# KinWaiCheuk/ReconVAT

Hardware: AMD Instinct MI355X
Metric: training audio-sec/sec (node) (higher is better)
Workload: dtype f32; 1 GPU; ReconVAT UNet_Onset VAT=True reconstruction=True, per-GPU B_l=8 + B_ul=8 segments of 327680 samples (640 frames x 229 mel), Adam+StepLR, fp32; parallelism=dp1, hipgraph=True, two_stream_schedule=True, kernel_plan_table=644fe159bb9eb70e, kernel_plan_mode=table, vat_nan_flag=0

## Files before the change

reconvat_amd/csrc/bn.hip:

```cpp
#include "common.h"

#define BN_PIX_PER_THREAD 16

__device__ __forceinline__ float bn_momentum_update(float running, float batch, float momentum) {
    return __fmaf_rn(momentum, batch, __fmul_rn(1.f - momentum, running));
}

struct BnArgs {
    const float* z; int z_ld;
    const float* dy; int dy_ld;
    float* out; int out_ld;
    const float* res; int res_ld;
    const float* r1_x; int r1_x_ld; const float* r1_w; const float* r1_b; int sk_cin, sk_ks;
    long P; int C;
    double* sums;
    const float* coef;
    float slope;
    int frozen;
    float* dgamma; float* dbeta;
    int accumulate;
    int param_accumulate;
    const float* gamma; const float* beta;
    float* running_mean; float* running_var; long* nbt;
    float* coef_out;
    float momentum, eps;
    int training;
    int ppt;
};

template <bool BWD>
__global__ __launch_bounds__(256) void bn_reduce_k(BnArgs a) {
    __shared__ float sh[256 * 8];
    const int C = a.C, C4 = C >> 2, PL = 256 / C4;
    const int t = threadIdx.x;
    const int c = (t % C4) * 4, pl = t / C4;
    f32x4 s0 = (f32x4){0.f, 0.f, 0.f, 0.f}, s1 = (f32x4){0.f, 0.f, 0.f, 0.f};
    if (pl < PL) {
        const long p0 = (long)blockIdx.x * PL * a.ppt;
        f32x4 mean, invstd, scale, shift;
        if (BWD) {
            mean = *reinterpret_cast<const f32x4*>(a.coef + c);
            invstd = *reinterpret_cast<const f32x4*>(a.coef + C + c);
            scale = *reinterpret_cast<const f32x4*>(a.coef + 2 * C + c);
            shift = *reinterpret_cast<const f32x4*>(a.coef + 3 * C + c);
        }
        for (int k = 0; k < a.ppt; k += 4) {
            f32x4 zv[4], dv[4];
            bool ok[4];
#pragma unroll
            for (int u = 0; u < 4; ++u) {
                const long p = p0 + pl + (long)(k + u) * PL;
                ok[u] = p < a.P;
                const long pp = ok[u] ? p : 0;
                zv[u] = *reinterpret_cast<const f32x4*>(a.z + pp * a.z_ld + c);
                if (BWD) dv[u] = *reinterpret_cast<const f32x4*>(a.dy + pp * a.dy_ld + c);
            }
#pragma unroll
            for (int u = 0; u < 4; ++u) {
                if (!ok[u]) continue;
                const f32x4 z = zv[u];
                if (BWD) {
                    const f32x4 d = dv[u];
#pragma unroll
                    for (int q = 0; q < 4; ++q) {
                        float zh = fmaf(z[q], scale[q], shift[q]);
                        float dd = zh > 0.f ? d[q] : d[q] * a.slope;
                        s0[q] += dd;
                        s1[q] += dd * ((z[q] - mean[q]) * invstd[q]);
                    }
                } else {
                    s0 += z;
#pragma unroll
                    for (int q = 0; q < 4; ++q) s1[q] = fmaf(z[q], z[q], s1[q]);
                }
            }
        }
    }
    if (pl < PL) {
#pragma unroll
        for (int q = 0; q < 4; ++q) {
            sh[(pl * C + c + q) * 2] = s0[q];
            sh[(pl * C + c + q) * 2 + 1] = s1[q];
        }
    }
    __syncthreads();
    if (t < 2 * C) {
        const int ch = t >> 1, which = t & 1;
        double d = 0.0;
        for (int l = 0; l < PL; ++l) d += (double)sh[(l * C + ch) * 2 + which];
        atomicAdd(&a.sums[(blockIdx.x % RV_BN_NREP) * 2 * C + which * C + ch], d);
    }
}

__device__ __forceinline__ void bn_coef(const BnArgs& a, const double* fold, int c, float& mean, float& invstd) {
    if (a.training) {
        const double n = (double)a.P;
        const double m = fold[c] / n;
        double var = fold[a.C + c] / n - m * m;
        if (var < 0.0) var = 0.0;
        mean = (float)m;
        invstd = (float)(1.0 / sqrt(var + (double)a.eps));
    } else {
        mean = a.running_mean[c];
        invstd = 1.0f / sqrtf(a.running_var[c] + a.eps);
    }
}

template <bool BWD, int SKIP = 0>
__global__ __launch_bounds__(256) void bn_apply_k(BnArgs a) {
    static_assert(!BWD || SKIP == 0, "the fused skip conv exists in the forward kernel only");
    extern __shared__ __attribute__((aligned(16))) float skw[];
    const int C = a.C, C4 = C >> 2;
    const long total = a.P * C4;
    const long stride = (long)gridDim.x * blockDim.x;
    long idx = (long)blockIdx.x * blockDim.x + threadIdx.x;
    const bool fixed = (stride % C4) == 0;
    int c = (int)(idx % C4) * 4;
    __shared__ double fold[256];
    if (BWD ? !a.frozen || a.dgamma : a.training) {
        for (int i = threadIdx.x; i < 2 * C; i += blockDim.x) fold[i] = bn_sum_replicas(a.sums, C, i);
        __syncthreads();
    }
    f32x4 mean, invstd, scale, shift, k1, k2;
    auto fetch = [&](int cc) {
        if (BWD) {
            scale = *reinterpret_cast<const f32x4*>(a.coef + 2 * C + cc);
            shift = *reinterpret_cast<const f32x4*>(a.coef + 3 * C + cc);
            mean = *reinterpret_cast<const f32x4*>(a.coef + cc);
            invstd = *reinterpret_cast<const f32x4*>(a.coef + C + cc);
            const double invn = 1.0 / (double)a.P;
#pragma unroll
            for (int q = 0; q < 4; ++q) {
                k1[q] = a.frozen ? 0.f : (float)(fold[cc + q] * invn);
                k2[q] = a.frozen ? 0.f : (float)(fold[C + cc + q] * invn);
            }
        } else {
#pragma unroll
            for (int q = 0; q < 4; ++q) {
                float m_, is_;
                bn_coef(a, fold, cc + q, m_, is_);
                scale[q] = a.gamma[cc + q] * is_;
                shift[q] = a.beta[cc + q] - m_ * scale[q];
            }
        }
    };
    fetch(c);
    f32x4 r1w = (f32x4){0.f, 0.f, 0.f, 0.f}, r1b = (f32x4){0.f, 0.f, 0.f, 0.f};
    auto fetch_r1 = [&](int cc) {
        if (!BWD && a.r1_x) {
            if (SKIP == 0) r1w = *reinterpret_cast<const f32x4*>(a.r1_w + cc);
            if (a.r1_b) r1b = *reinterpret_cast<const f32x4*>(a.r1_b + cc);
        }
    };
    fetch_r1(c);
    if constexpr (SKIP > 0) {
        for (int i = threadIdx.x; i < SKIP * C; i += blockDim.x) {
            const int cc = i / SKIP, kk = i - cc * SKIP;
            skw[kk * C + cc] = a.r1_w[i];
        }
        __syncthreads();
    }
    auto skip_dense = [&](const long p, const int cc0) -> f32x4 {
        constexpr int NCH = SKIP > 0 ? SKIP / 16 : 1;
        const float* xp = a.r1_x + p * a.r1_x_ld;
        auto chunk = [&](f32x4& acc, const int ch) {
            f32x4 xg[4];
#pragma unroll
            for (int g = 0; g < 4; ++g) xg[g] = *reinterpret_cast<const f32x4*>(xp + 16 * ch + 4 * g);
#pragma unroll
            for (int r = 0; r < 4; ++r)
#pragma unroll
                for (int g = 0; g < 4; ++g) {
                    const f32x4 w4 = *reinterpret_cast<const f32x4*>(&skw[(16 * ch + 4 * g + r) * C + cc0]);
#pragma unroll
                    for (int q = 0; q < 4; ++q) acc[q] = fmaf(w4[q], xg[g][r], acc[q]);
                }
        };
        f32x4 tot = (f32x4){0.f, 0.f, 0.f, 0.f};
        if (!a.sk_ks) {
#pragma unroll
            for (int ch = 0; ch < NCH; ++ch) chunk(tot, ch);
        } else {
#pragma unroll
            for (int w = 0; w < 4; ++w) {
                f32x4 part = (f32x4){0.f, 0.f, 0.f, 0.f};
                for (int ch = (w * NCH) / 4; ch < ((w + 1) * NCH) / 4; ++ch) chunk(part, ch);
                if (w == 0) tot = part; else tot += part;
            }
        }
        return tot + r1b;
    };
    auto one = [&](const f32x4& z, const f32x4& d, const f32x4& r) -> f32x4 {
        f32x4 o;
        if (!BWD) {
#pragma unroll
            for (int q = 0; q < 4; ++q) {
                float zh = fmaf(z[q], scale[q], shift[q]);
                o[q] = (zh > 0.f ? zh : zh * a.slope) + r[q];
            }
        } else {
#pragma unroll
            for (int q = 0; q < 4; ++q) {
                float zh = fmaf(z[q], scale[q], shift[q]);
                float dz = zh > 0.f ? d[q] : d[q] * a.slope;
                float xh = (z[q] - mean[q]) * invstd[q];
                dz = dz - k1[q] - xh * k2[q];
                o[q] = dz * scale[q];
            }
        }
        return o;
    };
    if (fixed) {
        constexpr int UNR = BWD || SKIP > 0 ? 4 : 8;
        const long pstep = stride / C4;
        long p = idx / C4;
        for (; p < a.P; p += UNR * pstep) {
            f32x4 zv[UNR], dv[UNR], rv[UNR];
            bool ok[UNR];
#pragma unroll
            for (int u = 0; u < UNR; ++u) {
                const long pu = p + u * pstep;
                ok[u] = pu < a.P;
                const long pp = ok[u] ? pu : 0;
                zv[u] = *reinterpret_cast<const f32x4*>(a.z + pp * a.z_ld + c);
                if (BWD) dv[u] = *reinterpret_cast<const f32x4*>(a.dy + pp * a.dy_ld + c);
                else dv[u] = (f32x4){0.f, 0.f, 0.f, 0.f};
                rv[u] = (f32x4){0.f, 0.f, 0.f, 0.f};
                if (!BWD && a.res) rv[u] = *reinterpret_cast<const f32x4*>(a.res + pp * a.res_ld + c);
                if (!BWD && SKIP == 0 && a.r1_x) {
                    const float x1 = a.r1_x[pp * a.r1_x_ld];
#pragma unroll
                    for (int q = 0; q < 4; ++q) rv[u][q] = fmaf(x1, r1w[q], r1b[q]);
                }
            }
            if constexpr (SKIP > 0) {
#pragma unroll
                for (int u = 0; u < UNR; ++u) rv[u] = skip_dense(ok[u] ? p + u * pstep : 0, c);
            }
#pragma unroll
            for (int u = 0; u < UNR; ++u) {
                if (!ok[u]) continue;
                f32x4 o = one(zv[u], dv[u], rv[u]);
                float* dst = a.out + (p + u * pstep) * a.out_ld + c;
                if (a.accumulate) {
                    f32x4 old = *reinterpret_cast<f32x4*>(dst);
                    o += old;
                }
                *reinterpret_cast<f32x4*>(dst) = o;
            }
        }
        idx = total;
    }
    for (; idx < total; idx += stride) {
        const long p = idx / C4;
        if (!fixed) { c = (int)(idx - p * C4) * 4; fetch(c); fetch_r1(c); }
        const f32x4 z = *reinterpret_cast<const f32x4*>(a.z + p * a.z_ld + c);
        f32x4 o;
        if (!BWD) {
            f32x4 r = (f32x4){0.f, 0.f, 0.f, 0.f};
            if (a.res) r = *reinterpret_cast<const f32x4*>(a.res + p * a.res_ld + c);
            if (SKIP == 0 && a.r1_x) {
                const float x1 = a.r1_x[p * a.r1_x_ld];
#pragma unroll
                for (int q = 0; q < 4; ++q) r[q] = fmaf(x1, r1w[q], r1b[q]);
            }
            if constexpr (SKIP > 0) r = skip_dense(p, c);
#pragma unroll
            for (int q = 0; q < 4; ++q) {
                float zh = fmaf(z[q], scale[q], shift[q]);
                o[q] = (zh > 0.f ? zh : zh * a.slope) + r[q];
            }
        } else {
            const f32x4 d = *reinterpret_cast<const f32x4*>(a.dy + p * a.dy_ld + c);
#pragma unroll
            for (int q = 0; q < 4; ++q) {
                float zh = fmaf(z[q], scale[q], shift[q]);
                float dz = zh > 0.f ? d[q] : d[q] * a.slope;
                float xh = (z[q] - mean[q]) * invstd[q];
                dz = dz - k1[q] - xh * k2[q];
                o[q] = dz * scale[q];
            }
        }
        float* dst = a.out + p * a.out_ld + c;
        if (a.accumulate) {
            f32x4 old = *reinterpret_cast<f32x4*>(dst);
            o += old;
        }
        *reinterpret_cast<f32x4*>(dst) = o;
    }
    if (blockIdx.x == 0) {
        for (int cc = threadIdx.x; cc < a.C; cc += blockDim.x) {
            if (BWD) {
                if (a.dgamma) {
                    const float dg = (float)fold[a.C + cc], db = (float)fold[cc];
                    a.dgamma[cc] = a.param_accumulate ? a.dgamma[cc] + dg : dg;
                    a.dbeta[cc] = a.param_accumulate ? a.dbeta[cc] + db : db;
                }
            } else {
                float m_, is_;
                bn_coef(a, fold, cc, m_, is_);
                const float sc = a.gamma[cc] * is_;
                a.coef_out[cc] = m_;
                a.coef_out[a.C + cc] = is_;
                a.coef_out[2 * a.C + cc] = sc;
                a.coef_out[3 * a.C + cc] = a.beta[cc] - m_ * sc;
                if (a.training) {
                    const double n = (double)a.P;
                    const double mm = fold[cc] / n;
                    double var = fold[a.C + cc] / n - mm * mm;
                    if (var < 0.0) var = 0.0;
                    const float unb = (float)(n > 1.0 ? var * n / (n - 1.0) : var);
                    a.coef_out[4 * a.C + cc] = unb;
                    if (a.training == 1) {
                        a.running_mean[cc] = bn_momentum_update(a.running_mean[cc], m_, a.momentum);
                        a.running_var[cc] = bn_momentum_update(a.running_var[cc], unb, a.momentum);
                    }
                }
            }
        }
        if (!BWD && threadIdx.x == 0 && a.training == 1 && a.nbt) *a.nbt += 1;
    }
}

static int bn_apply_blocks(long total, bool bwd = false) {
    long b = (total + 255) / 256;
    static const long capf = getenv("RV_BN_MAXBLK") ? atol(getenv("RV_BN_MAXBLK")) : 768;
    static const long capb = getenv("RV_BN_MAXBLK_BWD") ? atol(getenv("RV_BN_MAXBLK_BWD")) : 768;
    const long cap = bwd ? capb : capf;
    if (b > cap) b = cap;
    b = ((b + 2) / 3) * 3;
    return (int)b;
}

static int bn_ppt(long P, int PL) {
    long ppt = P / ((long)PL * 512);
    ppt = (ppt + 3) & ~3L;
    if (ppt < BN_PIX_PER_THREAD) ppt = BN_PIX_PER_THREAD;
    if (ppt > 256) ppt = 256;
    return (int)ppt;
}

int rv_internal_bn_stats(const float* z, int z_ld, long P, int C, double* sums, hipStream_t st) {
    RV_CHECK_ARG(C % 4 == 0 && C <= 128 && (z_ld % 4) == 0, "bn statistics: C=%d must be a multiple of 4 and <= 128", C);
    BnArgs a = {};
    a.z = z; a.z_ld = z_ld; a.P = P; a.C = C; a.sums = sums;
    const int PL = 256 / (C / 4);
    a.ppt = bn_ppt(P, PL);
    hipLaunchKernelGGL(bn_reduce_k<false>, dim3(cdiv(P, (long)PL * a.ppt)), dim3(256), 0, st, a);
    RV_LAUNCH_CHECK("bn statistics");
    return RV_OK;
}

int rv_internal_bn_bwd_stats(const float* dy, int dy_ld, const float* z, int z_ld, long P, int C, const float* coef, float slope,
                             double* sums, hipStream_t st) {
    RV_CHECK_ARG(C % 4 == 0 && C <= 128 && (z_ld % 4) == 0 && (dy_ld % 4) == 0, "bn backward statistics: C=%d unsupported", C);
    BnArgs a = {};
    a.z = z; a.z_ld = z_ld; a.dy = dy; a.dy_ld = dy_ld; a.P = P; a.C = C; a.sums = sums; a.coef = coef; a.slope = slope;
    const int PL = 256 / (C / 4);
    a.ppt = bn_ppt(P, PL);
    hipLaunchKernelGGL(bn_reduce_k<true>, dim3(cdiv(P, (long)PL * a.ppt)), dim3(256), 0, st, a);
    RV_LAUNCH_CHECK("bn backward statistics");
    return RV_OK;
}

extern "C" {

long rv_bn_workspace_bytes(int C) { return (long)RV_BN_NREP * (2 * C) * 8; }

int rv_bn_lrelu_fwd(const float* z, int z_ld, long P, int C, const float* gamma, const float* beta, float* running_mean,
                    float* running_var, long* num_batches_tracked, float momentum, float eps, int training, float slope,
                    const float* res, int res_ld, float* y, int y_ld, float* coef, void* workspace, int sums_ready,
                    void* stream) {
    hipStream_t st = (hipStream_t)stream;
    RV_CHECK_ARG(C % 4 == 0 && C <= 128, "rv_bn_lrelu_fwd: C=%d must be a multiple of 4 and <= 128", C);
    RV_CHECK_ARG((z_ld % 4) == 0 && (y_ld % 4) == 0 && (!res || (res_ld % 4) == 0), "rv_bn_lrelu_fwd: strides must be multiples of 4");
    BnArgs a = {};
    a.z = z; a.z_ld = z_ld; a.P = P; a.C = C; a.sums = (double*)workspace; a.slope = slope;
    a.gamma = gamma; a.beta = beta; a.running_mean = running_mean; a.running_var = running_var; a.nbt = num_batches_tracked;
    a.coef_out = coef; a.momentum = momentum; a.eps = eps; a.training = training;
    if (training && !sums_ready) {
        const int rc = rv_internal_bn_stats(z, z_ld, P, C, a.sums, st);
        if (rc != RV_OK) return rc;
    }
    a.out = y; a.out_ld = y_ld; a.res = res; a.res_ld = res_ld;
    hipLaunchKernelGGL(bn_apply_k<false>, dim3(bn_apply_blocks(P * (C / 4))), dim3(256), 0, st, a);
    RV_LAUNCH_CHECK("rv_bn_lrelu_fwd(apply)");
    return RV_OK;
}

int rv_bn_lrelu_fwd_skip(const float* z, int z_ld, long P, int C, const float* gamma, const float* beta, float* running_mean,
                         float* running_var, long* num_batches_tracked, float momentum, float eps, int training, float slope,
                         const float* x, int x_ld, int cin, const float* w, const float* b, int ksplit, float* y, int y_ld, float* coef,
                         void* workspace, int sums_ready, void* stream) {
    hipStream_t st = (hipStream_t)stream;
    RV_CHECK_ARG(C % 4 == 0 && C <= 128, "rv_bn_lrelu_fwd_skip: C=%d must be a multiple of 4 and <= 128", C);
    RV_CHECK_ARG(cin == 1 || cin == 16 || cin == 32 || cin == 64, "rv_bn_lrelu_fwd_skip: cin=%d (1, 16, 32 or 64)", cin);
    RV_CHECK_ARG((z_ld % 4) == 0 && (y_ld % 4) == 0 && x && w && x_ld >= cin && (cin == 1 || ((x_ld % 4) == 0 && (((uintptr_t)x) & 15) == 0)),
                 "rv_bn_lrelu_fwd_skip: bad strides / alignment / null skip operands");
    BnArgs a = {};
    a.z = z; a.z_ld = z_ld; a.P = P; a.C = C; a.sums = (double*)workspace; a.slope = slope;
    a.gamma = gamma; a.beta = beta; a.running_mean = running_mean; a.running_var = running_var; a.nbt = num_batches_tracked;
    a.coef_out = coef; a.momentum = momentum; a.eps = eps; a.training = training;
    if (training && !sums_ready) {
        const int rc = rv_internal_bn_stats(z, z_ld, P, C, a.sums, st);
        if (rc != RV_OK) return rc;
    }
    a.out = y; a.out_ld = y_ld; a.r1_x = x; a.r1_x_ld = x_ld; a.r1_w = w; a.r1_b = b; a.sk_cin = cin; a.sk_ks = ksplit;
    const dim3 grid(bn_apply_blocks(P * (C / 4)));
    const size_t lds = (size_t)cin * C * sizeof(float);
    if (cin == 1) hipLaunchKernelGGL((bn_apply_k<false, 0>), grid, dim3(256), 0, st, a);
    else if (cin == 16) hipLaunchKernelGGL((bn_apply_k<false, 16>), grid, dim3(256), lds, st, a);
    else if (cin == 32) hipLaunchKernelGGL((bn_apply_k<false, 32>), grid, dim3(256), lds, st, a);
    else hipLaunchKernelGGL((bn_apply_k<false, 64>), grid, dim3(256), lds, st, a);
    RV_LAUNCH_CHECK("rv_bn_lrelu_fwd_skip(apply)");
    return RV_OK;
}

int rv_bn_lrelu_bwd(const float* dy, int dy_ld, const float* z, int z_ld, long P, int C, const float* coef, float slope,
                    int frozen, float* dz, int dz_ld, float* dgamma, float* dbeta, int param_accumulate, void* workspace,
                    int sums_ready, void* stream) {
    hipStream_t st = (hipStream_t)stream;
    RV_CHECK_ARG(C % 4 == 0 && C <= 128, "rv_bn_lrelu_bwd: C=%d must be a multiple of 4 and <= 128", C);
    BnArgs a = {};
    a.z = z; a.z_ld = z_ld; a.dy = dy; a.dy_ld = dy_ld; a.P = P; a.C = C; a.sums = (double*)workspace;
    a.coef = coef; a.slope = slope; a.frozen = frozen; a.out = dz; a.out_ld = dz_ld; a.dgamma = dgamma; a.dbeta = dbeta; a.param_accumulate = param_accumulate;
    if ((!frozen || dgamma) && !sums_ready) {
        const int rc = rv_internal_bn_bwd_stats(dy, dy_ld, z, z_ld, P, C, coef, slope, a.sums, st);
        if (rc != RV_OK) return rc;
    }
    hipLaunchKernelGGL(bn_apply_k<true>, dim3(bn_apply_blocks(P * (C / 4), true)), dim3(256), 0, st, a);
    RV_LAUNCH_CHECK("rv_bn_lrelu_bwd(apply)");
    return RV_OK;
}

__global__ void bn_running_update_k(float* rm, float* rv, long* nbt, const float* coef, int C, float momentum) {
    int c = blockIdx.x * blockDim.x + threadIdx.x;
    if (c == 0 && nbt) *nbt += 1;
    if (c >= C) return;
    rm[c] = bn_momentum_update(rm[c], coef[c], momentum);
    rv[c] = bn_momentum_update(rv[c], coef[4 * C + c], momentum);
}

__global__ __launch_bounds__(128) void bn_running_update_table_k(const long* table, int nlayers, float momentum) {
    const long* e = table + (long)blockIdx.x * 6;
    float* rm = (float*)e[0];
    float* rv = (float*)e[1];
    long* nbt = (long*)e[2];
    const int C = (int)e[3];
    const long first = e[4], count = e[5];
    const long* coefs = table + (long)nlayers * 6 + first;
    for (int c = threadIdx.x; c < C; c += blockDim.x) {
        float m = rm[c], v = rv[c];
        for (long k = 0; k < count; ++k) {
            const float* coef = (const float*)coefs[k];
            m = bn_momentum_update(m, coef[c], momentum);
            v = bn_momentum_update(v, coef[4 * C + c], momentum);
        }
        rm[c] = m; rv[c] = v;
    }
    if (threadIdx.x == 0 && nbt) *nbt += count;
}

int rv_bn_running_update_table(const long* table, int nlayers, float momentum, void* stream) {
    RV_CHECK_ARG(table && nlayers > 0, "rv_bn_running_update_table: empty table");
    hipLaunchKernelGGL(bn_running_update_table_k, dim3(nlayers), dim3(128), 0, (hipStream_t)stream, table, nlayers, momentum);
    RV_LAUNCH_CHECK("rv_bn_running_update_table");
    return RV_OK;
}

int rv_bn_running_update(float* running_mean, float* running_var, long* num_batches_tracked, const float* coef, int C,
                         float momentum, void* stream) {
    hipLaunchKernelGGL(bn_running_update_k, dim3(cdiv(C, 128)), dim3(128), 0, (hipStream_t)stream, running_mean, running_var,
                       num_batches_tracked, coef, C, momentum);
    RV_LAUNCH_CHECK("rv_bn_running_update");
    return RV_OK;
}

}
```

Measured before the change: 16560 audio-s/s.

## Overlap BN apply prologue with first tile loads via per-channel coefficient table

Restructures the BN apply kernel prologue. The first unrolled batch of activation loads is issued before the replica-sum reduction, and one thread per channel computes scale/shift (or k1/k2) once into an LDS table instead of every thread recomputing them per channel. Block 0 can also finalize coef_out and running stats early, and the residual and skip variants become template parameters to remove runtime branches. The cost is raw s_barrier inline asm and more register pressure from holding the loads live across the reduction.

```diff
diff --git a/reconvat_amd/csrc/bn.hip b/reconvat_amd/csrc/bn.hip
--- a/reconvat_amd/csrc/bn.hip
+++ b/reconvat_amd/csrc/bn.hip
@@ -92,65 +92,70 @@
     }
 }
 
-__device__ __forceinline__ void bn_coef(const BnArgs& a, const double* fold, int c, float& mean, float& invstd) {
+__device__ __forceinline__ void bn_coef(const BnArgs& a, double sum, double sumsq, float rmean, float rvar, float& mean, float& invstd) {
     if (a.training) {
         const double n = (double)a.P;
-        const double m = fold[c] / n;
-        double var = fold[a.C + c] / n - m * m;
+        const double m = sum / n;
+        double var = sumsq / n - m * m;
         if (var < 0.0) var = 0.0;
         mean = (float)m;
         invstd = (float)(1.0 / sqrt(var + (double)a.eps));
     } else {
-        mean = a.running_mean[c];
-        invstd = 1.0f / sqrtf(a.running_var[c] + a.eps);
-    }
-}
-
-template <bool BWD, int SKIP = 0>
+        mean = rmean;
+        invstd = 1.0f / sqrtf(rvar + a.eps);
+    }
+}
+
+#ifndef RV_BN_HEAD
+#define RV_BN_HEAD 3
+#endif
+
+template <bool BWD, int SKIP = 0, int RES = 0>
 __global__ __launch_bounds__(256) void bn_apply_k(BnArgs a) {
-    static_assert(!BWD || SKIP == 0, "the fused skip conv exists in the forward kernel only");
+    static_assert(!BWD || (SKIP == 0 && RES == 0), "residual and fused skip conv exist in the forward kernel only");
+    static_assert(SKIP == 0 || RES == 0, "the dense skip conv is the residual");
+    constexpr bool HOIST = (RV_BN_HEAD & 1) != 0, EARLY = (RV_BN_HEAD & 2) != 0;
     extern __shared__ __attribute__((aligned(16))) float skw[];
+    __shared__ double fold[256];
+    __shared__ __attribute__((aligned(16))) float ctab[256];
     const int C = a.C, C4 = C >> 2;
     const long total = a.P * C4;
     const long stride = (long)gridDim.x * blockDim.x;
     long idx = (long)blockIdx.x * blockDim.x + threadIdx.x;
     const bool fixed = (stride % C4) == 0;
     int c = (int)(idx % C4) * 4;
-    __shared__ double fold[256];
-    if (BWD ? !a.frozen || a.dgamma : a.training) {
-        for (int i = threadIdx.x; i < 2 * C; i += blockDim.x) fold[i] = bn_sum_replicas(a.sums, C, i);
-        __syncthreads();
+    const int tc = threadIdx.x;
+    const bool coef_thread = tc < C;
+    const bool sums = BWD ? !a.frozen || a.dgamma : a.training != 0;
+    double rep[RV_BN_NREP];
+    float gam = 0.f, bet = 0.f, rmean = 0.f, rvar = 0.f;
+    if (sums && tc < 2 * C) {
+#pragma unroll
+        for (int r = 0; r < RV_BN_NREP; ++r) rep[r] = a.sums[r * 2 * C + tc];
+    }
+    if (!BWD && coef_thread) {
+        gam = a.gamma[tc];
+        bet = a.beta[tc];
+        if (!a.training) { rmean = a.running_mean[tc]; rvar = a.running_var[tc]; }
     }
     f32x4 mean, invstd, scale, shift, k1, k2;
-    auto fetch = [&](int cc) {
+    auto fetch_saved = [&](int cc) {
         if (BWD) {
             scale = *reinterpret_cast<const f32x4*>(a.coef + 2 * C + cc);
             shift = *reinterpret_cast<const f32x4*>(a.coef + 3 * C + cc);
             mean = *reinterpret_cast<const f32x4*>(a.coef + cc);
             invstd = *reinterpret_cast<const f32x4*>(a.coef + C + cc);
-            const double invn = 1.0 / (double)a.P;
-#pragma unroll
-            for (int q = 0; q < 4; ++q) {
-                k1[q] = a.frozen ? 0.f : (float)(fold[cc + q] * invn);
-                k2[q] = a.frozen ? 0.f : (float)(fold[C + cc + q] * invn);
-            }
-        } else {
-#pragma unroll
-            for (int q = 0; q < 4; ++q) {
-                float m_, is_;
-                bn_coef(a, fold, cc + q, m_, is_);
-                scale[q] = a.gamma[cc + q] * is_;
-                shift[q] = a.beta[cc + q] - m_ * scale[q];
-            }
-        }
-    };
-    fetch(c);
+        }
+    };
+    auto fetch_table = [&](int cc) {
+        const f32x4 t0 = *reinterpret_cast<const f32x4*>(&ctab[cc]), t1 = *reinterpret_cast<const f32x4*>(&ctab[C + cc]);
+        if (BWD) { k1 = t0; k2 = t1; } else { scale = t0; shift = t1; }
+    };
+    fetch_saved(c);
     f32x4 r1w = (f32x4){0.f, 0.f, 0.f, 0.f}, r1b = (f32x4){0.f, 0.f, 0.f, 0.f};
     auto fetch_r1 = [&](int cc) {
-        if (!BWD && a.r1_x) {
-            if (SKIP == 0) r1w = *reinterpret_cast<const f32x4*>(a.r1_w + cc);
-            if (a.r1_b) r1b = *reinterpret_cast<const f32x4*>(a.r1_b + cc);
-        }
+        if (RES == 2) r1w = *reinterpret_cast<const f32x4*>(a.r1_w + cc);
+        if ((RES == 2 || SKIP > 0) && a.r1_b) r1b = *reinterpret_cast<const f32x4*>(a.r1_b + cc);
     };
     fetch_r1(c);
     if constexpr (SKIP > 0) {
@@ -158,8 +163,8 @@
             const int cc = i / SKIP, kk = i - cc * SKIP;
             skw[kk * C + cc] = a.r1_w[i];
         }
-        __syncthreads();
-    }
+    }
+    asm volatile("" ::: "memory");
     auto skip_dense = [&](const long p, const int cc0) -> f32x4 {
         constexpr int NCH = SKIP > 0 ? SKIP / 16 : 1;
         const float* xp = a.r1_x + p * a.r1_x_ld;
@@ -210,116 +215,149 @@
         }
         return o;
     };
-    if (fixed) {
-        constexpr int UNR = BWD || SKIP > 0 ? 4 : 8;
-        const long pstep = stride / C4;
-        long p = idx / C4;
-        for (; p < a.P; p += UNR * pstep) {
-            f32x4 zv[UNR], dv[UNR], rv[UNR];
-            bool ok[UNR];
+    constexpr int UNR = BWD || SKIP > 0 ? 4 : 8;
+    const long pstep = stride / C4;
+    long p = idx / C4;
+    f32x4 zv[UNR], dv[UNR], rv[UNR];
+    bool ok[UNR];
+    auto load_trip = [&]() __attribute__((always_inline)) {
+#pragma unroll
+        for (int u = 0; u < UNR; ++u) {
+            const long pu = p + u * pstep;
+            ok[u] = pu < a.P;
+            const long pp = ok[u] ? pu : 0;
+            zv[u] = *reinterpret_cast<const f32x4*>(a.z + pp * a.z_ld + c);
+            if (BWD) dv[u] = *reinterpret_cast<const f32x4*>(a.dy + pp * a.dy_ld + c);
+            else dv[u] = (f32x4){0.f, 0.f, 0.f, 0.f};
+            rv[u] = (f32x4){0.f, 0.f, 0.f, 0.f};
+            if (RES == 1) rv[u] = *reinterpret_cast<const f32x4*>(a.res + pp * a.res_ld + c);
+            if (RES == 2) rv[u][0] = a.r1_x[pp * a.r1_x_ld];
+        }
+    };
+    auto finish_trip = [&]() __attribute__((always_inline)) {
+        if (RES == 2) {
 #pragma unroll
             for (int u = 0; u < UNR; ++u) {
-                const long pu = p + u * pstep;
-                ok[u] = pu < a.P;
-                const long pp = ok[u] ? pu : 0;
-                zv[u] = *reinterpret_cast<const f32x4*>(a.z + pp * a.z_ld + c);
-                if (BWD) dv[u] = *reinterpret_cast<const f32x4*>(a.dy + pp * a.dy_ld + c);
-                else dv[u] = (f32x4){0.f, 0.f, 0.f, 0.f};
-                rv[u] = (f32x4){0.f, 0.f, 0.f, 0.f};
-                if (!BWD && a.res) rv[u] = *reinterpret_cast<const f32x4*>(a.res + pp * a.res_ld + c);
-                if (!BWD && SKIP == 0 && a.r1_x) {
-                    const float x1 = a.r1_x[pp * a.r1_x_ld];
-#pragma unroll
-                    for (int q = 0; q < 4; ++q) rv[u][q] = fmaf(x1, r1w[q], r1b[q]);
+                const float x1 = rv[u][0];
+#pragma unroll
+                for (int q = 0; q < 4; ++q) rv[u][q] = fmaf(x1, r1w[q], r1b[q]);
+            }
+        }
+        if constexpr (SKIP > 0) {
+#pragma unroll
+            for (int u = 0; u < UNR; ++u) rv[u] = skip_dense(ok[u] ? p + u * pstep : 0, c);
+        }
+#pragma unroll
+        for (int u = 0; u < UNR; ++u) {
+            if (!ok[u]) continue;
+            f32x4 o = one(zv[u], dv[u], rv[u]);
+            float* dst = a.out + (p + u * pstep) * a.out_ld + c;
+            if (a.accumulate) {
+                f32x4 old = *reinterpret_cast<f32x4*>(dst);
+                o += old;
+            }
+            *reinterpret_cast<f32x4*>(dst) = o;
+        }
+    };
+    double s0 = 0.0, s1 = 0.0;
+    auto finalize = [&]() {
+        if (BWD) {
+            if (a.dgamma) {
+                const float dg = (float)s1, db = (float)s0;
+                a.dgamma[tc] = a.param_accumulate ? a.dgamma[tc] + dg : dg;
+                a.dbeta[tc] = a.param_accumulate ? a.dbeta[tc] + db : db;
+            }
+        } else {
+            float m_, is_;
+            bn_coef(a, s0, s1, rmean, rvar, m_, is_);
+            const float sc = gam * is_;
+            a.coef_out[tc] = m_;
+            a.coef_out[C + tc] = is_;
+            a.coef_out[2 * C + tc] = sc;
+            a.coef_out[3 * C + tc] = bet - m_ * sc;
+            if (a.training) {
+                const double n = (double)a.P;
+                const double mm = s0 / n;
+                double var = s1 / n - mm * mm;
+                if (var < 0.0) var = 0.0;
+                const float unb = (float)(n > 1.0 ? var * n / (n - 1.0) : var);
+                a.coef_out[4 * C + tc] = unb;
+                if (a.training == 1) {
+                    a.running_mean[tc] = bn_momentum_update(a.running_mean[tc], m_, a.momentum);
+                    a.running_var[tc] = bn_momentum_update(a.running_var[tc], unb, a.momentum);
                 }
             }
-            if constexpr (SKIP > 0) {
-#pragma unroll
-                for (int u = 0; u < UNR; ++u) rv[u] = skip_dense(ok[u] ? p + u * pstep : 0, c);
-            }
-#pragma unroll
-            for (int u = 0; u < UNR; ++u) {
-                if (!ok[u]) continue;
-                f32x4 o = one(zv[u], dv[u], rv[u]);
-                float* dst = a.out + (p + u * pstep) * a.out_ld + c;
-                if (a.accumulate) {
-                    f32x4 old = *reinterpret_cast<f32x4*>(dst);
-                    o += old;
+            if (tc == 0 && a.training == 1 && a.nbt) *a.nbt += 1;
+        }
+    };
+    auto head = [&]() __attribute__((always_inline)) {
+        if (sums) {
+            if (tc < 2 * C) {
+                double s = 0.0;
+#pragma unroll
+                for (int r = 0; r < RV_BN_NREP; ++r) {
+                    asm volatile("" : "+v"(rep[r]));
+                    s += rep[r];
                 }
-                *reinterpret_cast<f32x4*>(dst) = o;
-            }
-        }
-        idx = total;
-    }
-    for (; idx < total; idx += stride) {
-        const long p = idx / C4;
-        if (!fixed) { c = (int)(idx - p * C4) * 4; fetch(c); fetch_r1(c); }
-        const f32x4 z = *reinterpret_cast<const f32x4*>(a.z + p * a.z_ld + c);
-        f32x4 o;
-        if (!BWD) {
-            f32x4 r = (f32x4){0.f, 0.f, 0.f, 0.f};
-            if (a.res) r = *reinterpret_cast<const f32x4*>(a.res + p * a.res_ld + c);
-            if (SKIP == 0 && a.r1_x) {
-                const float x1 = a.r1_x[p * a.r1_x_ld];
-#pragma unroll
-                for (int q = 0; q < 4; ++q) r[q] = fmaf(x1, r1w[q], r1b[q]);
-            }
-            if constexpr (SKIP > 0) r = skip_dense(p, c);
-#pragma unroll
-            for (int q = 0; q < 4; ++q) {
-                float zh = fmaf(z[q], scale[q], shift[q]);
-                o[q] = (zh > 0.f ? zh : zh * a.slope) + r[q];
-            }
-        } else {
-            const f32x4 d = *reinterpret_cast<const f32x4*>(a.dy + p * a.dy_ld + c);
-#pragma unroll
-            for (int q = 0; q < 4; ++q) {
-                float zh = fmaf(z[q], scale[q], shift[q]);
-                float dz = zh > 0.f ? d[q] : d[q] * a.slope;
-                float xh = (z[q] - mean[q]) * invstd[q];
-                dz = dz - k1[q] - xh * k2[q];
-                o[q] = dz * scale[q];
-            }
-        }
-        float* dst = a.out + p * a.out_ld + c;
-        if (a.accumulate) {
-            f32x4 old = *reinterpret_cast<f32x4*>(dst);
-            o += old;
-        }
-        *reinterpret_cast<f32x4*>(dst) = o;
-    }
-    if (blockIdx.x == 0) {
-        for (int cc = threadIdx.x; cc < a.C; cc += blockDim.x) {
+                fold[tc] = s;
+            }
+            asm volatile("s_waitcnt lgkmcnt(0)\n\ts_barrier" ::: "memory");
+            if (coef_thread) { s0 = fold[tc]; s1 = fold[C + tc]; }
+        }
+        if (coef_thread) {
             if (BWD) {
-                if (a.dgamma) {
-                    const float dg = (float)fold[a.C + cc], db = (float)fold[cc];
-                    a.dgamma[cc] = a.param_accumulate ? a.dgamma[cc] + dg : dg;
-                    a.dbeta[cc] = a.param_accumulate ? a.dbeta[cc] + db : db;
-                }
+                const double invn = 1.0 / (double)a.P;
+                ctab[tc] = a.frozen ? 0.f : (float)(s0 * invn);
+                ctab[C + tc] = a.frozen ? 0.f : (float)(s1 * invn);
             } else {
                 float m_, is_;
-                bn_coef(a, fold, cc, m_, is_);
-                const float sc = a.gamma[cc] * is_;
-                a.coef_out[cc] = m_;
-                a.coef_out[a.C + cc] = is_;
-                a.coef_out[2 * a.C + cc] = sc;
-                a.coef_out[3 * a.C + cc] = a.beta[cc] - m_ * sc;
-                if (a.training) {
-                    const double n = (double)a.P;
-                    const double mm = fold[cc] / n;
-                    double var = fold[a.C + cc] / n - mm * mm;
-                    if (var < 0.0) var = 0.0;
-                    const float unb = (float)(n > 1.0 ? var * n / (n - 1.0) : var);
-                    a.coef_out[4 * a.C + cc] = unb;
-                    if (a.training == 1) {
-                        a.running_mean[cc] = bn_momentum_update(a.running_mean[cc], m_, a.momentum);
-                        a.running_var[cc] = bn_momentum_update(a.running_var[cc], unb, a.momentum);
-                    }
-                }
-            }
-        }
-        if (!BWD && threadIdx.x == 0 && a.training == 1 && a.nbt) *a.nbt += 1;
-    }
+                bn_coef(a, s0, s1, rmean, rvar, m_, is_);
+                const float sc = gam * is_;
+                ctab[tc] = sc;
+                ctab[C + tc] = bet - m_ * sc;
+            }
+            if (EARLY && blockIdx.x == 0) finalize();
+        }
+        asm volatile("s_waitcnt lgkmcnt(0)\n\ts_barrier" ::: "memory");
+    };
+    if (fixed && a.P > 0) {
+        if (HOIST) load_trip();
+        asm volatile("" ::: "memory");
+        head();
+        fetch_table(c);
+        if (!HOIST) load_trip();
+        for (;;) {
+            finish_trip();
+            p += UNR * pstep;
+            if (p >= a.P) break;
+            load_trip();
+        }
+    } else {
+        head();
+        for (; idx < total; idx += stride) {
+            const long pg = idx / C4;
+            c = (int)(idx - pg * C4) * 4;
+            fetch_saved(c); fetch_table(c); fetch_r1(c);
+            const f32x4 z = *reinterpret_cast<const f32x4*>(a.z + pg * a.z_ld + c);
+            f32x4 d = (f32x4){0.f, 0.f, 0.f, 0.f}, r = (f32x4){0.f, 0.f, 0.f, 0.f};
+            if (BWD) d = *reinterpret_cast<const f32x4*>(a.dy + pg * a.dy_ld + c);
+            if (RES == 1) r = *reinterpret_cast<const f32x4*>(a.res + pg * a.res_ld + c);
+            if (RES == 2) {
+                const float x1 = a.r1_x[pg * a.r1_x_ld];
+#pragma unroll
+                for (int q = 0; q < 4; ++q) r[q] = fmaf(x1, r1w[q], r1b[q]);
+            }
+            if constexpr (SKIP > 0) r = skip_dense(pg, c);
+            f32x4 o = one(z, d, r);
+            float* dst = a.out + pg * a.out_ld + c;
+            if (a.accumulate) {
+                f32x4 old = *reinterpret_cast<f32x4*>(dst);
+                o += old;
+            }
+            *reinterpret_cast<f32x4*>(dst) = o;
+        }
+    }
+    if (!EARLY && blockIdx.x == 0 && coef_thread) finalize();
 }
 
 static int bn_apply_blocks(long total, bool bwd = false) {
@@ -383,7 +421,9 @@
         if (rc != RV_OK) return rc;
     }
     a.out = y; a.out_ld = y_ld; a.res = res; a.res_ld = res_ld;
-    hipLaunchKernelGGL(bn_apply_k<false>, dim3(bn_apply_blocks(P * (C / 4))), dim3(256), 0, st, a);
+    const dim3 grid(bn_apply_blocks(P * (C / 4)));
+    if (res) hipLaunchKernelGGL((bn_apply_k<false, 0, 1>), grid, dim3(256), 0, st, a);
+    else hipLaunchKernelGGL((bn_apply_k<false, 0, 0>), grid, dim3(256), 0, st, a);
     RV_LAUNCH_CHECK("rv_bn_lrelu_fwd(apply)");
     return RV_OK;
 }
@@ -408,7 +448,7 @@
     a.out = y; a.out_ld = y_ld; a.r1_x = x; a.r1_x_ld = x_ld; a.r1_w = w; a.r1_b = b; a.sk_cin = cin; a.sk_ks = ksplit;
     const dim3 grid(bn_apply_blocks(P * (C / 4)));
     const size_t lds = (size_t)cin * C * sizeof(float);
-    if (cin == 1) hipLaunchKernelGGL((bn_apply_k<false, 0>), grid, dim3(256), 0, st, a);
+    if (cin == 1) hipLaunchKernelGGL((bn_apply_k<false, 0, 2>), grid, dim3(256), 0, st, a);
     else if (cin == 16) hipLaunchKernelGGL((bn_apply_k<false, 16>), grid, dim3(256), lds, st, a);
     else if (cin == 32) hipLaunchKernelGGL((bn_apply_k<false, 32>), grid, dim3(256), lds, st, a);
     else hipLaunchKernelGGL((bn_apply_k<false, 64>), grid, dim3(256), lds, st, a);
```

Result: no change. 16710 audio-s/s, median of 6 (+0.9%).
